# AI4REALNET/network-distributed-q-learning

Hardware: NVIDIA B200
Metric: switch_agent_decisions_per_sec (higher is better)
Workload: dtype f64

## Files before the change

network-distributed-q-learning_b200/csrc/sfl_core.cuh:

```cuda
#pragma once
#include <stdint.h>
#include "switchfl_b200.h"

#if defined(__CUDACC__) && !defined(SFL_HOST_EMUL)
#define SFL_DEV 1
#define SFL_FN __device__ __forceinline__
#define SFL_NI __device__ __forceinline__
#define SFL_RARE __device__ __noinline__
#define SFL_NU _Pragma("unroll 1")
#define SFL_U4 _Pragma("unroll 4")
#define SFL_UA _Pragma("unroll")
#else
#define SFL_DEV 0
#include <math.h>
#include <string.h>
#define SFL_FN inline
#define SFL_NI inline
#define SFL_RARE inline
#define SFL_NU
#define SFL_U4
#define SFL_UA
struct int4 { int x, y, z, w; };
struct int2 { int x, y; };
static inline int4 make_int4(int x, int y, int z, int w) { int4 r = {x, y, z, w}; return r; }
// ... 101 lines not shown
  RO<int> dist;
  RO<int8_t> qinit;
};

struct Layout {
  int T, S, NP, NT, a_max, q_cap, q_stride, pend_cap;
  unsigned off_tra, off_trb, off_pend, off_sem, off_rewards, off_sws, off_q;
  unsigned off_rng;
  unsigned long long env_stride;
};

struct EnvHdr {
  int elapsed, episode, step_counter, num_malf;
  int terminated, truncated, need_reset, halted;
  int err, q_rows, pending_fin, cur_dec;
  int act_cursor, ev_cursor, n_dec_logged, n_tick_logged;
  int n_ep_logged, q_init_on, aborted, cur_train;
  unsigned long long active_mask, malf_prev_mask, at_dest_mask, done_mask;
  unsigned long long decisions, ticks, train_ticks;
  double cum_reward;
  int last_next_sw;
  int eps_tag;
  unsigned eps_z, eps_w;
  unsigned long long forced_stops, stop_actions, arrived_trains;
  int dec_t, dec_go;
  unsigned long long ph[6], ph_t0;
};

struct SwS { int ninter, pad; double eps_pow; };
enum { HM_ACTIVE = 0, HM_MALF = 1, HM_DEST = 2, HM_DONE = 3 };

struct RunArgs {
  int mode, max_ticks, n_envs, trace_sem;
  int dec_cap, tick_cap, ep_cap, act_cap, ev_cap, max_steps, q_init_on, phase_clock;
  unsigned hot_bytes, env_smem, tail_hot, pad2;
  char *state;
  const sfl_hparams *hp;
  sfl_env_counters *counters;
  sfl_dec_rec *trace_dec; sfl_tick_rec *trace_tick; int4 *trace_sem_buf;
  sfl_ep_rec *ep_log; int *ep_delay;
  sfl_step_rec *step_out;
  double *sq_q; long long *sq_d; int *sq_c;
  const int8_t *replay_act; const int *replay_ev;
  const double *eval_q;
};

struct KArgs { DevMap m; Layout L; RunArgs ra; };
#define SFL_K const KArgs &K
#define c_m (K.m)
#define c_L (K.L)
#define c_ra (K.ra)

#if SFL_DEV
extern __shared__ __align__(16) char g_smem[];
typedef unsigned hot_t;
SFL_FN char *hot_ptr(hot_t o) { return g_smem + o; }
#else
typedef char *hot_t;
SFL_FN char *hot_ptr(hot_t o) { return o; }
#endif

template <bool TH, bool SQ_ = false> struct EnvT {
  static const bool SQ = SQ_;
  static const bool EVQ = false;
  static const bool HOT_TAIL = TH;
  static const int NW = 1;
  const KArgs *kp;
  hot_t hot;
  char *gb;
  SFL_FN EnvHdr *h() const { return (EnvHdr *)hot_ptr(hot); }
  SFL_FN int4 *tra() const { return (int4 *)(hot_ptr(hot) + kp->L.off_tra); }
  SFL_FN int4 *trb() const { return (int4 *)(hot_ptr(hot) + kp->L.off_trb); }
  SFL_FN char *tail() const { return TH ? hot_ptr(hot) : gb; }
  SFL_FN int2 *pend() const { return (int2 *)(tail() + kp->L.off_pend); }
  SFL_FN int4 *sem() const { return (int4 *)(tail() + kp->L.off_sem); }
  SFL_FN int *rewards() const { return (int *)(tail() + kp->L.off_rewards); }
  SFL_FN SwS *sws() const { return (SwS *)(tail() + kp->L.off_sws); }
  SFL_FN double *q() const { return (double *)(gb + kp->L.off_q); }
  hot_t own;
  SFL_FN uint8_t *own_ptr() const { return (uint8_t *)hot_ptr(own); }
  SFL_FN int owner(int p) const { return TH ? sem()[p].z : (int)(int8_t)own_ptr()[p]; }
  SFL_FN void sem_put(int p, int4 r) const { sem()[p] = r; if (!TH) own_ptr()[p] = (uint8_t)r.z; }
  SFL_FN void sem_drop(int p) const { sem()[p].z = -1; if (!TH) own_ptr()[p] = 0xFFu; }
  SFL_FN unsigned long long &hw0(int m) const {
    EnvHdr *x = h();
    return m == HM_ACTIVE ? x->active_mask : m == HM_MALF ? x->malf_prev_mask : m == HM_DEST ? x->at_dest_mask : x->done_mask;
  }
  SFL_FN unsigned long long *hw1(int m) const { return (unsigned long long *)(hot_ptr(hot) + sizeof(EnvHdr)) + m; }
};
template <bool TH, bool SQ_ = false> struct EnvW : EnvT<TH, SQ_> { static const int NW = 2; };
template <class Base> struct EnvEval : Base { static const bool EVQ = true; };
template <bool TH, bool SQ, int NW, bool EVQ = false> struct EnvOf { typedef EnvT<TH, SQ> type; };
template <bool TH, bool SQ> struct EnvOf<TH, SQ, 2, false> { typedef EnvW<TH, SQ> type; };
template <bool TH, int NW> struct EnvOf<TH, false, NW, true> { typedef EnvEval<typename EnvOf<TH, false, NW>::type> type; };

template <class Env> SFL_FN TSet<Env::NW> tset(const Env &e, int m) {
  TSet<Env::NW> s; s.w[0] = e.hw0(m); if (Env::NW > 1) s.w[Env::NW - 1] = *e.hw1(m); return s;
}
template <class Env> SFL_FN void tset_put(const Env &e, int m, const TSet<Env::NW> &s) { e.hw0(m) = s.w[0]; if (Env::NW > 1) *e.hw1(m) = s.w[Env::NW - 1]; }
template <class Env> SFL_FN int tset_any(const Env &e, int m) { return Env::NW == 1 ? e.hw0(m) != 0ull : (e.hw0(m) | *e.hw1(m)) != 0ull; }
template <class Env> SFL_FN int tset_pop(const Env &e, int m) { TSet<Env::NW> s = tset(e, m); const int t = s.pop(); tset_put(e, m, s); return t; }
template <class Env> SFL_FN void tset_add(const Env &e, int m, int t) {
  if (Env::NW > 1 && t >= 64) *e.hw1(m) |= 1ull << (t & 63); else e.hw0(m) |= 1ull << t;
}



struct Scratch {
  const KArgs *kp;
  hot_t base;
  SFL_FN int4 *tmp() const { return (int4 *)hot_ptr(base); }
  SFL_FN int4 *rng() const { return (int4 *)(hot_ptr(base) + 16 * kp->L.T); }
  SFL_FN int *inj() const { return (int *)(hot_ptr(base) + 16 * kp->L.T); }
  SFL_FN int8_t *occ() const { return (int8_t *)(hot_ptr(base) + 32 * kp->L.T); }
  SFL_FN uint8_t *blk() const { return (uint8_t *)(hot_ptr(base) + 33 * kp->L.T); }
};
#if SFL_DEV
__host__
#endif
SFL_FN unsigned scratch_bytes(int T) { return (unsigned)(32 * T + ((2 * T + 15) / 16) * 16); }

struct Hp {
  hot_t o;
  SFL_FN const sfl_hparams *operator->() const { return (const sfl_hparams *)hot_ptr(o); }
};

#if SFL_DEV
SFL_FN unsigned long long sm_clock() { return (unsigned long long)clock64(); }
#else
SFL_FN unsigned long long sm_clock() { return 0ull; }
#endif
enum { PH_TICK = 0, PH_OBSERVE = 1, PH_ACT = 2, PH_APPLY = 3, PH_UPDATE = 4, PH_RESET = 5 };
#define SFL_PHASE_START(h) do { if (TRACE && c_ra.phase_clock) (h)->ph_t0 = sm_clock(); } while (0)
#define SFL_PHASE_MARK(h, i) do { if (TRACE && c_ra.phase_clock) { const unsigned long long t_ = sm_clock(); (h)->ph[i] += t_ - (h)->ph_t0; (h)->ph_t0 = t_; } } while (0)

enum { K_LEARN = 0, K_GREEDY = 1, K_FULL = 2 };
template <int KIND> SFL_FN int run_mode(SFL_K) { return KIND == K_LEARN ? (int)SFL_MODE_LEARN : KIND == K_GREEDY ? (int)SFL_MODE_GREEDY : c_ra.mode; }

struct U4 { unsigned x, y, z, w; };
SFL_FN unsigned mulhi32(unsigned a, unsigned b) { return (unsigned)(((unsigned long long)a * b) >> 32); }
SFL_FN U4 philox4x32(unsigned c0, unsigned c1, unsigned c2, unsigned c3, unsigned k0, unsigned k1) {
  SFL_NU
  for (int i = 0; i < 10; i++) {
    unsigned h0 = mulhi32(0xD2511F53u, c0), l0 = 0xD2511F53u * c0;
    unsigned h1 = mulhi32(0xCD9E8D57u, c2), l1 = 0xCD9E8D57u * c2;
    unsigned n0 = h1 ^ c1 ^ k0, n2 = h0 ^ c3 ^ k1;
    c0 = n0; c1 = l1; c2 = n2; c3 = l0;
    k0 += 0x9E3779B9u; k1 += 0xBB67AE85u;
  }
  U4 r = {c0, c1, c2, c3};
  return r;
}

struct Pcg {
  unsigned long long s_hi, s_lo, i_hi, i_lo;
  unsigned has32, u32, pad0, pad1;
};
#define SFL_PCG_BYTES 48

SFL_FN void pcg_step(Pcg &g) {
  const unsigned long long M_HI = 0x2360ED051FC65DA4ull, M_LO = 0x4385DF649FCCF645ull;
  const unsigned long long lo = g.s_lo * M_LO;
  const unsigned long long hi = mulhi64(g.s_lo, M_LO) + g.s_lo * M_HI + g.s_hi * M_LO;
  g.s_lo = lo + g.i_lo;
  g.s_hi = hi + g.i_hi + (g.s_lo < lo ? 1ull : 0ull);
}
// ... 88 lines not shown
#define SFL_MT_N 624
#define SFL_MT_M 397
SFL_FN unsigned mt_temper(unsigned y) {
  y ^= y >> 11;
  y ^= (y << 7) & 0x9D2C5680u;
  y ^= (y << 15) & 0xEFC60000u;
  return y ^ (y >> 18);
}
template <int G> SFL_FN int mt_seed(unsigned *key, unsigned long long seed, const Grp<G> &g) {
  if (seed >> 32) return 0;
  if (g.gl == 0) {
    unsigned s = (unsigned)seed;
    SFL_NU
    for (int i = 0; i < SFL_MT_N; i++) { key[i] = s; s = 1812433253u * (s ^ (s >> 30)) + (unsigned)(i + 1); }
  }
  g.sync();
  return 1;
}
template <int G> SFL_FN void mt_twist(unsigned *key, unsigned *out, const Grp<G> &g) {
  SFL_NU
  for (int base = 0; base < SFL_MT_N; base += G) {
    const int i = base + g.gl;
    unsigned v = 0u;
    if (i < SFL_MT_N) {
      const unsigned y = (key[i] & 0x80000000u) | (key[i + 1 == SFL_MT_N ? 0 : i + 1] & 0x7FFFFFFFu);
      v = key[i < SFL_MT_N - SFL_MT_M ? i + SFL_MT_M : i - (SFL_MT_N - SFL_MT_M)] ^ (y >> 1) ^ ((0u - (y & 1u)) & 0x9908B0DFu);
    }
    g.sync();
    if (i < SFL_MT_N) key[i] = v;
    g.sync();
  }
  for (int i = g.gl; i < SFL_MT_N; i += G) out[i] = mt_temper(key[i]);
  g.sync();
}
template <int G> SFL_FN unsigned mt_next(unsigned *key, unsigned *out, int &pos, const Grp<G> &g) {
  if (pos == SFL_MT_N) { mt_twist(key, out, g); pos = 0; }
  return out[pos++];
}
template <int G> SFL_FN unsigned mt_masked(unsigned *key, unsigned *out, int &pos, const Grp<G> &g, unsigned rng) {
  if (!rng) return 0u;
  unsigned mask = rng;
  mask |= mask >> 1; mask |= mask >> 2; mask |= mask >> 4; mask |= mask >> 8; mask |= mask >> 16;
  unsigned v;
  SFL_NU
  do v = mt_next(key, out, pos, g) & mask; while (v > rng);
  return v;
}
template <int G> SFL_FN int malf_schedule_env(unsigned long long seed, unsigned long long hit_below, int lo, int hi, int T, int steps,
                                              int *ev, int ev_cap, unsigned *key, unsigned *out, const Grp<G> &g) {
  if (!mt_seed(key, seed, g)) return -1;
  int n = 0, pos = SFL_MT_N;
  const unsigned rng = (unsigned)hi - (unsigned)lo;
  SFL_NU
  for (int tick = 1; hit_below && tick <= steps; tick++) {
    SFL_NU
    for (int t = 0; t < T; t++) {
      const unsigned a = mt_next(key, out, pos, g), b = mt_next(key, out, pos, g);
      if ((((unsigned long long)(a >> 5) << 26) | (b >> 6)) >= hit_below) continue;
      const int dur = lo + (int)mt_masked(key, out, pos, g, rng) + 1;
      if (g.gl == 0 && n < ev_cap) { ev[3 * n] = tick; ev[3 * n + 1] = t; ev[3 * n + 2] = dur; }
      n++;
    }
  }
  if (g.gl == 0 && n < ev_cap) ev[3 * n] = -1;
  return n;
}

struct Mv { int cell, dir, valid; };
SFL_FN unsigned mv_entry(SFL_K, int cell, int dir) { return c_m.move[(size_t)cell * 4 + dir]; }
SFL_FN int mv_valid(unsigned e, int action) { return (e >> (3 * action)) & 1; }
SFL_FN Mv mv_apply(SFL_K, unsigned e, int action, int cell) {
  unsigned f = (e >> (3 * action)) & 7u;
  int nd = (int)(f >> 1);
  int delta = (nd & 1) ? (2 - nd) : (nd - 1) * c_m.Wp;
  Mv r;
  r.cell = (e & 0x8000u) ? cell + delta : cell;
  r.dir = nd; r.valid = (int)(f & 1u);
  return r;
}
SFL_FN Mv check_action(SFL_K, int action, int cell, int dir) { return mv_apply(K, mv_entry(K, cell, dir), action, cell); }

SFL_FN int is_moving(int a) { return a >= A_LEFT && a <= A_RIGHT; }

template <class Env>
SFL_FN int tr_state(Env e, int t) { return (e.tra()[t].y >> 8) & 0xFF; }
template <class Env>
SFL_FN int rule_port(Env e, int port, int me, int now, int blocking_type) {
  int4 r;
  if (Env::HOT_TAIL) {
    r = e.sem()[port];
    if (r.z < 0 || r.z == me || r.x > now || r.x + r.y < now) return 0;
  } else {
    const int holder = e.owner(port);
    if (holder < 0 || holder == me) return 0;
    r = e.sem()[port];
    if (r.x > now || r.x + r.y < now) return 0;
  }
  if (r.w == blocking_type) return 1;
  return tr_state(e, r.z) == ST_MALF;
}
template <class Env>
SFL_FN int port_blocked(Env e, int next_port, int out_port, int me, int now) {
  if (next_port >= 0) {
    if (rule_port(e, next_port, me, now, SEM_OUT)) return 1;
    return rule_port(e, out_port, me, now, SEM_IN);
  }
  return rule_port(e, out_port, me, now, SEM_OUT);
}

template <class Env>
SFL_RARE void q_insert(SFL_K, Env e, const Hp hp, unsigned key, double *row) {
  *(unsigned long long *)row = (unsigned long long)key + 1ull;
  e.h()->q_rows++;
  unsigned per_port = (unsigned)(c_L.NT * 48);
  int port = (int)(key / per_port);
  int A = c_m.sw[c_m.port[port].w].y;
  double dq = hp->default_q;
  SFL_NU
  for (int a = 0; a < A; a++) row[1 + a] = dq;
  if (c_ra.q_init_on) {
    unsigned rem = key - (unsigned)port * per_port;
    int tgt = (int)(rem / 48u), semb = (int)((rem % 48u) / 3u);
    int qi = c_m.qinit[port * c_L.NT + tgt];
    if (qi >= 0 && semb != 0) row[1 + (qi & 15)] = (qi & 16) ? 1000.0 : 500.0;
  }
}

template <class Env>
SFL_NI double *q_row(SFL_K, Env e, const Hp hp, unsigned key) {
  if (Env::SQ) return c_ra.sq_q + (size_t)key * c_L.a_max;
  unsigned mask = (unsigned)c_L.q_cap - 1u;
  unsigned i = (key * 2654435761u) >> 7;
  SFL_NU
  for (int probe = 0; probe < c_L.q_cap; probe++) {
    i &= mask;
    double *row = e.q() + (size_t)i * c_L.q_stride;
    unsigned long long k = *(unsigned long long *)row;
    if (k == (unsigned long long)key + 1ull) return row + 1;
    if (k == 0ull) {
      if (e.h()->q_rows >= c_L.q_cap - 1) break;
      q_insert(K, e, hp, key, row);
      return row + 1;
    }
    i++;
  }
  e.h()->err |= SFL_ERR_Q_FULL;
  return e.q() + 1;
}

#if SFL_DEV
SFL_FN void shared_add(long long *d, int *c, long long v) { atomicAdd((unsigned long long *)d, (unsigned long long)v); atomicAdd(c, 1); }
#else
SFL_FN void shared_add(long long *d, int *c, long long v) { *d += v; *c += 1; }
#endif

SFL_FN double lr_pow(double rate, int n) {
  double r = 1.0, b = rate;
  SFL_NU
  for (; n > 0; n >>= 1) { if (n & 1) r = dmul(r, b); b = dmul(b, b); }
  return r;
}

SFL_FN double td_value(double q, double lr, double reward, double gamma, double mq, int bootstrap) {
  const double one_m = dadd(1.0, -lr);
  return bootstrap ? dadd(dmul(one_m, q), dmul(lr, dadd(reward, dmul(gamma, mq)))) : dadd(dmul(one_m, q), dmul(lr, reward));
}

template <class Env>
SFL_NI void q_update(SFL_K, Env e, const Hp hp, unsigned key, int action, double reward,
                     const double *next_row, int prev_sw, int next_sw) {
  double *row = q_row(K, e, hp, key);
  double lr = hp->lr;
  if (hp->lr_decay_rate != 1.0) lr = dmul(lr, lr_pow(hp->lr_decay_rate, e.sws()[prev_sw].ninter));
  const double q = row[action];
  double mq = 0.0;
  if (next_sw != prev_sw && next_row) {
    int A = c_m.sw[next_sw].y;
    mq = next_row[0];
    SFL_NU
    for (int a = 1; a < A; a++) { const double v = next_row[a]; mq = v > mq ? v : mq; }
// ... 73 lines not shown
      if (r.z < 0 || r.x > now) e.sem()[unique] = make_int4(now, d_ot, h, SEM_OUT);
      if (far_port != source && far_port != out_port && far_port != unique) {
        r = e.sem()[far_port];
        if (r.z < 0 || r.w == SEM_IN || r.x > now) e.sem()[far_port] = make_int4(now, d_ot + up.y + 1, h, SEM_IN);
      }
    }
    if (target != source && target != out_port) {
      r = e.sem()[target];
      if (r.z < 0 || r.w == SEM_OUT || r.x > now) e.sem()[target] = make_int4(now, d_ot + 1, h, SEM_OUT);
    }
  } else {
    int4 r;
    if (e.owner(out_port) < 0) e.sem_put(out_port, make_int4(now, 3, h, SEM_OUT));
    else { r = e.sem()[out_port]; if (r.w == SEM_OUT || r.x > now) e.sem_put(out_port, make_int4(now, 3, h, r.w)); }
    int d_ot = c_m.port[out_port].y;
    if (e.owner(target) < 0) e.sem_put(target, make_int4(now, d_ot + 1, h, SEM_IN));
    else { r = e.sem()[target]; if (r.w == SEM_IN || r.x > now) e.sem_put(target, make_int4(now, d_ot + 1, h, r.w)); }
    int unique = c_m.port[target].z;
    if (unique >= 0) {
      int4 up = c_m.port[unique];
      int far_port = up.x;
      if (unique != source && unique != out_port && unique != target) {
        r = e.sem()[unique];
        if (e.owner(unique) < 0 || r.w == SEM_OUT || r.x > now) e.sem_put(unique, make_int4(now, d_ot + 1, h, SEM_OUT));
      }
      r = e.sem()[unique];
      if (e.owner(unique) < 0 || r.x > now) e.sem_put(unique, make_int4(now, d_ot, h, SEM_OUT));
      if (far_port != source && far_port != out_port && far_port != unique) {
        r = e.sem()[far_port];
        if (e.owner(far_port) < 0 || r.w == SEM_IN || r.x > now) e.sem_put(far_port, make_int4(now, d_ot + up.y + 1, h, SEM_IN));
      }
    }
    if (target != source && target != out_port) {
      r = e.sem()[target];
      if (e.owner(target) < 0 || r.w == SEM_OUT || r.x > now) e.sem_put(target, make_int4(now, d_ot + 1, h, SEM_OUT));
    }
  }
}

template <class Env>
SFL_FN int delay_at(SFL_K, Env e, int tgt_index, int cell, int dir, int now, int la) {
  int d = c_m.dist[((size_t)tgt_index * (c_m.Hp * c_m.Wp) + cell) * 4 + dir];
  if (d >= SFL_INF_DIST) { e.h()->err |= SFL_ERR_INF_DISTANCE; d = 0; }
  return now - la + d;
}

template <int KIND, class Env>
SFL_FN void finish_decision(SFL_K, Env e, const Hp hp, int env_id) {
  const bool TRACE = KIND == K_FULL;
  const int mode = run_mode<KIND>(K);
  EnvHdr *h = e.h();
  SFL_PHASE_START(h);
  if (mode == SFL_MODE_LEARN || mode == SFL_MODE_REPLAY) {
    TSet<Env::NW> fresh = tset(e, HM_DONE).andnot(tset(e, HM_DEST));
    SFL_NU
    while (fresh.any()) {
      int t = fresh.pop();
      tset_add(e, HM_DEST, t);
      int4 b = e.trb()[t];
      int n = (b.y >> 16) & 0xFF;
      SFL_NU
      for (int i = 0; i < n; i++) {
        int2 pe = e.pend()[t * c_L.pend_cap + i];
        q_update(K, e, hp, (unsigned)pe.x, (pe.y >> 24) & 15, 1000.0, nullptr, (pe.y >> 12) & 0xFFF, -1);
      }
      b.y &= 0xFFFF;
      e.trb()[t] = b;
    }
    SwS *ss = e.sws() + h->pending_fin;
    ss->ninter++;
    ss->eps_pow = dmul(ss->eps_pow, hp->epsilon_decay_rate);
  }
  h->pending_fin = -1;
  SFL_PHASE_MARK(h, PH_UPDATE);
  if (h->step_counter > c_ra.max_steps) h->truncated = 1;
  if (TRACE) {
    if (c_ra.trace_dec && h->cur_dec >= 0 && h->cur_dec < c_ra.dec_cap) {
      sfl_dec_rec *rec = c_ra.trace_dec + (size_t)env_id * c_ra.dec_cap + h->cur_dec;
      rec->arrived = h->done_mask; rec->arrived_hi = Env::NW > 1 ? *e.hw1(HM_DONE) : 0ull;
      rec->done = h->terminated | (h->truncated << 1);
      if (c_ra.trace_sem_buf) {
        int4 *dst = c_ra.trace_sem_buf + ((size_t)env_id * c_ra.dec_cap + h->cur_dec) * c_L.NP;
        SFL_NU
        for (int p = 0; p < c_L.NP; p++) { int4 r = e.sem()[p]; r.y += r.x; dst[p] = r; }
      }
    }
    h->cur_dec = -1;
  }
}

template <int G, class Env>
SFL_FN int observe_bits(SFL_K, Env e, const Grp<G> &g, const int on, const int t) {
  const int now = e.h()->elapsed;
  const int s = on ? (e.trb()[t].y & 0xFFFF) : 0;
  const int4 sw = c_m.sw[s];
  unsigned bits = 0;
  SFL_UA
  for (int base = 0; base < 8; base += G) {
    const int j = base + g.gl;
    int b = 0;
    if (on && j < 8 && (j & 3) < sw.x) {
      const int port = sw.z + (j & 3);
      b = (j & 4) ? rule_port(e, port, t, now, SEM_IN) : rule_port(e, c_m.port[port].x, t, now, SEM_OUT);
    }
    bits |= (g.ballot(b) & 0xFFu) << base;
  }
  return (int)(~(bits | (bits >> 4)) & ((1u << sw.x) - 1u));
}

struct Obs { int s, P, A, p0, a0, cur, semb, mask, ok; unsigned key; };
template <class Env>
SFL_FN Obs observe(SFL_K, Env e, int t, int now, const int4 ta, const int4 tb, const int semb_pre = -1) {
  Obs ob;
  ob.s = tb.y & 0xFFFF;
  const int4 sw = c_m.sw[ob.s];
  ob.P = sw.x; ob.A = sw.y; ob.p0 = sw.z; ob.a0 = sw.w;
  const int4 tr0 = c_m.train0[t], tr1 = c_m.train1[t];
  const int my_port = (int)((unsigned)ta.w >> 16);
  const int dist_now = c_m.dist[((size_t)tr0.w * (c_m.Hp * c_m.Wp) + ta.x) * 4 + (ta.y & 0xFF)];
  int semb = semb_pre;
  if (semb_pre < 0) {
    semb = 0;
    SFL_NU
    for (int k = 0; k < ob.P; k++)
      if (!port_blocked(e, c_m.port[ob.p0 + k].x, ob.p0 + k, t, now)) semb |= 1 << k;
  }
  ob.semb = semb;
  ob.cur = my_port - ob.p0;
  ob.ok = ob.cur >= 0 && ob.cur < ob.P;
  ob.key = 0u; ob.mask = 0;
  if (!ob.ok) return ob;
  int delay = now - tr1.y + dist_now;
  if (dist_now >= SFL_INF_DIST) { e.h()->err |= SFL_ERR_INF_DISTANCE; delay = now - tr1.y; }
  int level = delay <= 0 ? 0 : (delay <= (tr1.y - tr1.x) * 20 ? 1 : 2);
  ob.key = (((unsigned)(ob.p0 + ob.cur) * c_L.NT + tr0.w) * 16u + semb) * 3u + level;
  const int4 px = c_m.pexit[ob.p0 + ob.cur];
  int mask = 1 << (ob.A - 1);
  {
    int ex[3] = {px.y, px.z, px.w};
#if SFL_DEV
#pragma unroll
#endif
    for (int i = 0; i < 3; i++) if (i < px.x && ((semb >> ((ex[i] >> 4) & 3)) & 1)) mask |= 1 << (ex[i] & 15);
  }
  ob.mask = mask;
  return ob;
}

template <int KIND, class Env>
SFL_FN void decide(SFL_K, Env e, const Hp hp, int env_id, int t, const int semb_pre = -1) {
  const bool TRACE = KIND == K_FULL;
  const int mode = run_mode<KIND>(K);
  EnvHdr *h = e.h();
  const int now = h->elapsed;
  SFL_PHASE_START(h);
  int4 ta = e.tra()[t], tb = e.trb()[t];
  const int learning = mode == SFL_MODE_LEARN || mode == SFL_MODE_REPLAY;
  const int s_early = tb.y & 0xFFFF;
  const int reward_in = e.rewards()[s_early * c_L.T + t];
  double eps_pow = 1.0;
  int ninter = 0;
  if (mode == SFL_MODE_LEARN) {
    eps_pow = e.sws()[s_early].eps_pow;
    if (KIND == K_FULL && c_L.off_rng) ninter = e.sws()[s_early].ninter;
  }
  int2 pend0 = make_int2(0, -1);
  if (learning && ((tb.y >> 16) & 0xFF)) pend0 = e.pend()[t * c_L.pend_cap];
// ... 77 lines not shown
    if (pl >= SFL_PLAN_CAP) { h->err |= SFL_ERR_PLAN_FULL; pl = SFL_PLAN_CAP - 1; }
    plan = ((plan << 4) | A_STOP) & 0xFFFFu; pl++;
  } else { plan = A_FWD | ((unsigned)move2 << 4); pl = 2; }
  ta.z = (int)plan | (pl << 16);
  e.tra()[t] = ta;
  int all_blocked = 1;
  if ((plan & 0xFu) == A_STOP) {
    if (moving) all_blocked = port_blocked(e, next_port, out_port, t, now);
    else all_blocked = (mask == (1 << (A - 1)));
  }
  int cell = pos, d2 = dir;
  {
    unsigned pp = plan;
    SFL_NU
    for (int i = 0; i < pl; i++, pp >>= 4) {
      int a = pp & 0xF;
      if (a != A_STOP) { Mv c = check_action(K, a, cell, d2); cell = c.cell; d2 = c.dir; }
    }
  }
  int curr = delay_at(K, e, tr0.w, cell, d2, now, tr1.y);
  int reward_out = tb.z - curr;
  if (!all_blocked && (plan & 0xFu) == A_STOP) reward_out -= 1300;
  e.rewards()[next_switch * c_L.T + t] = reward_out;
  tb.z = curr;
  h->step_counter++;
  SFL_PHASE_MARK(h, PH_APPLY);
  if (learning) {
    int n = (tb.y >> 16) & 0xFF;
    int2 *pend = e.pend() + t * c_L.pend_cap;
    int hit = -1, same = -1;
    SFL_NU
    for (int i = 0; i < n; i++) {
      int nsw = (i ? pend[i].y : pend0.y) & 0xFFF;
      if (nsw == s && hit < 0) hit = i;
    }
    if (hit >= 0) {
      int2 pe = hit ? pend[hit] : pend0;
      const int prev_sw = (pe.y >> 12) & 0xFFF;
      if (prev_sw != s && !my_row) my_row = q_row(K, e, hp, key);
      q_update(K, e, hp, (unsigned)pe.x, (pe.y >> 24) & 15, (double)reward_in, my_row, prev_sw, s);
      SFL_NU
      for (int j = hit; j + 1 < n; j++) pend[j] = pend[j + 1];
      n--;
    }
    int meta = next_switch | (s << 12) | (action << 24);
    SFL_NU
    for (int i = 0; i < n; i++) if ((pend[i].y & 0xFFF) == next_switch) same = i;
    if (same >= 0) pend[same] = make_int2((int)key, meta);
    else if (n >= c_L.pend_cap) h->err |= SFL_ERR_PEND_FULL;
    else { pend[n] = make_int2((int)key, meta); n++; }
    tb.y = (tb.y & 0xFFFF) | (n << 16);
  }
  e.trb()[t] = tb;
  SFL_PHASE_MARK(h, PH_UPDATE);
  h->cum_reward += (double)reward_in;
  if (TRACE) {
    if (c_ra.trace_dec) {
      h->cur_dec = h->n_dec_logged;
      if (h->n_dec_logged < c_ra.dec_cap) {
        sfl_dec_rec *rec = c_ra.trace_dec + (size_t)env_id * c_ra.dec_cap + h->n_dec_logged;
        rec->ep = h->episode; rec->tick = now; rec->sw = s; rec->train = t; rec->key = key; rec->mask = mask;
        rec->action = action; rec->next_sw = next_switch; rec->reward = reward_in; rec->done = 0; rec->arrived = 0;
        rec->arrived_hi = 0;
      }
      h->n_dec_logged++;
    }
  }
  if (TRACE) h->last_next_sw = next_switch;
  h->decisions++;
  if (mask == (1 << (A - 1))) h->forced_stops++;
  if (action == A - 1) h->stop_actions++;
  h->pending_fin = s;
}

template <int G, class Env>
SFL_RARE void env_reset(SFL_K, Env e, const Grp<G> &g, int on) {
  EnvHdr *h = e.h();
  const int T = on ? c_L.T : 0, NP = on ? c_L.NP : 0;
  SFL_NU
  for (int t = g.gl; t < T; t += G) {
    int4 tr0 = c_m.train0[t], tr1 = c_m.train1[t];
    e.tra()[t] = make_int4(-1, tr0.y | (ST_WAITING << 8) | (0 << 16) | (A_NONE << 24), 0, (int)((unsigned)tr1.z << 16));
    int4 b = e.trb()[t];
    e.trb()[t] = make_int4(b.x, 0xFFFF, c_m.init_delay[t], 0);
  }
  SFL_NU
  for (int p = g.gl; p < NP; p += G) e.sem_put(p, make_int4(0, 0, -1, 0));
  SFL_NU
  for (int i = g.gl; i < c_L.S * T; i += G) e.rewards()[i] = 0;
  g.sync();
  if (on && g.gl == 0) {
    SFL_NU
    for (int t = 0; t < T; t++) {
      int4 tr1 = c_m.train1[t];
      e.sem_put(tr1.z, make_int4(tr1.x - 2, tr1.w + 2, t, SEM_IN));
    }
    h->elapsed = 0; h->step_counter = 0; h->num_malf = 0; h->terminated = 0; h->truncated = 0; h->need_reset = 0;
    h->pending_fin = -1; h->cur_dec = -1; h->ev_cursor = 0; h->active_mask = 0; h->malf_prev_mask = 0; h->at_dest_mask = 0;
    h->eps_tag = -1;
    h->done_mask = 0; h->cum_reward = 0.0;
    if (Env::NW > 1) { SFL_UA for (int m = 0; m < 4; m++) *e.hw1(m) = 0ull; }
  }
  g.sync();
}

template <int NW> struct TickRegs {
  int elapsed, ended, rng_blk;
  TSet<NW> active, done;
  unsigned ticks, train_ticks;
};

SFL_FN int malf_stage2(const Hp hp, int now, int t) {
  const U4 u = philox4x32((unsigned)now, (unsigned)t, 0xA11Eu, 0u, (unsigned)hp->seed, (unsigned)(hp->seed >> 32));
  if (u.x >= hp->malf_thr2) return 0;
  return hp->malf_min + (int)(((unsigned long long)u.y * (unsigned)(hp->malf_max - hp->malf_min + 1)) >> 32) + 1;
}

template <int G, int KIND, bool ONE, class Env>
SFL_FN void env_tick(SFL_K, Env e, Scratch sc, const Hp hp, int env_id, const Grp<G> &g, TickRegs<Env::NW> &R, const int live) {
  const bool TRACE = KIND == K_FULL;
  EnvHdr *h = e.h();
  const int Tw = c_L.T;
  const int T = live ? Tw : 0;
  const int now = R.elapsed + 1;
  const int replay_ev = KIND != K_LEARN && c_ra.replay_ev != 0;
  const unsigned thr = live ? hp->malf_threshold : 0u;
  if (replay_ev) {
    SFL_NU
    for (int t = g.gl; t < T; t += G) sc.inj()[t] = 0;
    g.sync();
    if (live && g.gl == 0) {
      const int *ev = c_ra.replay_ev + (size_t)env_id * c_ra.ev_cap * 3;
      int c = h->ev_cursor;
      SFL_NU
      while (c < c_ra.ev_cap && ev[c * 3] >= 0 && ev[c * 3] <= now) { if (ev[c * 3] == now) sc.inj()[ev[c * 3 + 1]] = ev[c * 3 + 2]; c++; }
      h->ev_cursor = c;
    }
    g.sync();
  }
  const int fresh_rng = !replay_ev && thr && (now >> 4) != R.rng_blk;
  const unsigned coarse = (thr >> 24) + ((thr & 0xFFFFFFu) ? 1u : 0u);
  SFL_NU
  for (int t = g.gl, once_ = 1; t < T && (!ONE || once_); t += G, once_ = 0) {
    int4 ta = e.tra()[t];
    const int p = ta.x, d = ta.y & 0xFF, st = (ta.y >> 8) & 0xFF;
    int saved = (ta.y >> 16) & 0xFF, prev_act = (ta.y >> 24) & 0xFF;
    unsigned plan = (unsigned)ta.z & 0xFFFFu;
    int pl = ta.z >> 16, mc = ta.w & 0xFFFF;
    int dur = 0;
    if (replay_ev) dur = sc.inj()[t];
    else if (thr) {
      if (fresh_rng) {
        U4 u = philox4x32((unsigned)(now >> 4), (unsigned)t, 0xA11Fu, 0u, (unsigned)hp->seed, (unsigned)(hp->seed >> 32));
        sc.rng()[t] = make_int4((int)u.x, (int)u.y, (int)u.z, (int)u.w);
      }
      if (((const uint8_t *)&sc.rng()[t])[now & 15] < coarse) dur = malf_stage2(hp, now, t);
    }
    if (mc == 0 && dur > 0) mc = dur;
    int src, dst, ecell = -1, nd = d, act = A_NOTHING, a = A_NOTHING, flags = 0;
    if (st == ST_DONE) { src = dst = -1 - t; }
    else {
      int pp = p, dd = d;
      if (p < 0) { const int4 tr0 = c_m.train0[t]; pp = tr0.x; dd = tr0.y; }
      const unsigned me = mv_entry(K, pp, dd);
      if (pl == 0) a = A_FWD;
      else { a = plan & 0xF; prev_act = a; plan >>= 4; pl--; }
      if (p >= 0) { Mv c = mv_apply(K, me, a, p); ecell = c.valid ? c.cell : p; flags = 1 | (c.valid ? 2 : 0); }
      act = a;
      if (st == ST_WAITING) act = A_NOTHING;
      if ((act == A_LEFT || act == A_RIGHT) && !mv_valid(me, act)) act = A_FWD;
      if (is_moving(act) && !mv_valid(me, act)) act = A_STOP;
      if (is_moving(act) && !saved) saved = act;
      const int upd = (mc == 0) && act != A_STOP;
      int ncell = p;
      if (p < 0) { if (saved) { ncell = pp; nd = dd; } }
      else if (saved && upd) { Mv c = mv_apply(K, me, saved, p); if (c.valid) { ncell = c.cell; nd = c.dir; } act = saved; }
      src = p >= 0 ? p : -1 - t;
      dst = ncell >= 0 ? ncell : src;
    }
    ta.y = d | (st << 8) | (saved << 16) | (prev_act << 24);
    ta.z = (int)plan | (pl << 16);
    ta.w = (ta.w & (int)0xFFFF0000) | mc;
    e.tra()[t] = ta;
    sc.tmp()[t] = make_int4(src, dst, ecell, nd | (act << 8) | (a << 16) | (flags << 24));
  }
  if (fresh_rng) R.rng_blk = now >> 4;
  g.sync();
  TSet<Env::NW> chain;
  chain.clear();
  SFL_NU
  for (int base = 0; base < (ONE ? 1 : Tw); base += (ONE ? 1 : G)) {
    const int t = base + g.gl;
    int follows = 0;
    if (t < T) {
      int4 m = sc.tmp()[t];
      int s = m.x, d = m.y;
      int wants = d != s, blocked = !wants, occ = -1;
      if (wants) {
        SFL_NU
        for (int k = 0; k < T; k++) {
          const int2 o = *(const int2 *)&sc.tmp()[k];
          occ = o.x == d ? k : occ;
          blocked |= (o.y == d) & (o.y != o.x) & (k < t);
        }
        if (occ >= 0) { int2 o = *(const int2 *)&sc.tmp()[occ]; if (o.y == s && o.y != o.x) blocked = 1; }
      }
      sc.occ()[t] = (int8_t)occ; sc.blk()[t] = (uint8_t)blocked;
      follows = !blocked && occ >= 0;
    }
    chain.or_ballot(g.ballot(follows), base);
  }
  g.sync();
  if (g.wany(chain.any())) {
    SFL_NU
    for (int iter = 0; iter < Tw; iter++) {
      int changed = 0;
      if (chain.any()) {
        SFL_NU
        for (int t = g.gl, once_ = 1; t < T && (!ONE || once_); t += G, once_ = 0) {
          int occ = sc.occ()[t];
          if (!sc.blk()[t] && occ >= 0 && ((volatile uint8_t *)sc.blk())[occ]) { sc.blk()[t] = 1; changed = 1; }
        }
      }
      g.sync();
      if (!g.wany(changed)) break;
    }
  }
  TSet<Env::NW> done_bits, malf_bits, stopped_bits, depart_bits, active;
  done_bits.clear(); malf_bits.clear(); stopped_bits.clear(); depart_bits.clear(); active.clear();
  SFL_NU
  for (int base = 0; base < (ONE ? 1 : Tw); base += (ONE ? 1 : G)) {
    const int t = base + g.gl;
    int f_done = 0, f_malf = 0, f_stop = 0, f_dep = 0, f_act = 0;
    if (t < T) {
      int4 ta = e.tra()[t];
      const int4 m = sc.tmp()[t];
      int p = ta.x, d = ta.y & 0xFF;
      const int st = (ta.y >> 8) & 0xFF;
      int saved = (ta.y >> 16) & 0xFF;
      const int prev_act = (ta.y >> 24) & 0xFF;
      unsigned plan = (unsigned)ta.z & 0xFFFFu;
      int pl = ta.z >> 16, mc = ta.w & 0xFFFF, next_port = (int)((unsigned)ta.w >> 16);
      const int act = (m.w >> 8) & 0xFF, popped = (m.w >> 16) & 0xFF, fl = (m.w >> 24) & 0xFF;
      const int wants = m.y != m.x;
      const int in_malf = mc > 0, allowed = !in_malf && wants && !sc.blk()[t];
      const int4 tr0 = c_m.train0[t];
      const int ed = c_m.train1[t].x;
      const int ed_reached = now >= ed, stop_given = act == A_STOP, valid_move = is_moving(act) && allowed, conflict = !allowed;
      int nxt = st;
      switch (st) {
        case ST_WAITING: if (in_malf) nxt = ST_MALF_OFF; else if (ed_reached) nxt = ST_READY; break;
        case ST_READY: if (in_malf) nxt = ST_MALF_OFF; else if (valid_move) nxt = ST_MOVING; break;
        case ST_MALF_OFF:
          if (!in_malf) { if (ed_reached) nxt = valid_move ? ST_MOVING : ST_STOPPED; else nxt = ST_WAITING; }
          break;
        case ST_MOVING: if (in_malf) nxt = ST_MALF; else if (stop_given || conflict) nxt = ST_STOPPED; break;
        case ST_STOPPED: if (in_malf) nxt = ST_MALF; else if (valid_move) nxt = ST_MOVING; break;
        case ST_MALF: if (!in_malf && valid_move) nxt = ST_MOVING; else if (!in_malf && (stop_given || conflict)) nxt = ST_STOPPED; break;
        default: break;
      }
      if (nxt >= ST_MOVING && nxt <= ST_MALF) {
        if (st <= ST_MALF_OFF) { p = tr0.x; d = tr0.y; }
        else if (allowed) { p = m.y; d = m.w & 0xFF; if (p == tr0.z) nxt = ST_DONE; }
      }
      if (nxt == ST_DONE) p = -1;
      if (mc > 0) mc--;
      if (p >= 0) saved = 0;
      f_done = nxt == ST_DONE; f_malf = mc != 0; f_stop = nxt == ST_STOPPED || nxt == ST_MALF; f_dep = now == ed - 2;
      if (TRACE) {
        if (c_ra.trace_tick && h->n_tick_logged < c_ra.tick_cap) {
          sfl_tick_rec *rec = c_ra.trace_tick + ((size_t)env_id * c_ra.tick_cap + h->n_tick_logged) * T + t;
          rec->pos = p; rec->dir = (int8_t)d; rec->state = (int8_t)nxt; rec->malf = (int16_t)mc;
        }
      }
      if ((fl & 1) && (fl & 2) && m.z != p && popped != A_STOP) {
        if (pl >= SFL_PLAN_CAP) { h->err |= SFL_ERR_PLAN_FULL; pl = SFL_PLAN_CAP - 1; }
        plan = ((plan << 4) | (unsigned)popped) & 0xFFFFu; pl++;
        if (c_m.cell_switch[m.z] >= 0) {
          int src_port = (int)((unsigned)e.trb()[t].x >> 16);
          if (src_port != 0xFFFF) next_port = src_port;
        }
      }
      if (p >= 0 && nxt != ST_WAITING) {
        int peek = pl ? (int)(plan & 0xF) : A_FWD;
        Mv c = check_action(K, peek, p, d);
        int s = c_m.cell_switch[c.cell];
        if (s >= 0) {
          int ok = 1;
          if (nxt == ST_MOVING || nxt == ST_READY) { }
          else if ((nxt == ST_STOPPED || nxt == ST_MALF) && prev_act == A_STOP) { }
          else if (nxt == ST_STOPPED || nxt == ST_MALF) s = c_m.port[next_port].w;
          else ok = 0;
          if (ok) { ((uint16_t *)&e.trb()[t].y)[0] = (uint16_t)s; f_act = 1; }
        }
      }
      ta.x = p;
      ta.y = d | (nxt << 8) | (saved << 16) | (prev_act << 24);
      ta.z = (int)plan | (pl << 16);
      ta.w = mc | (next_port << 16);
      e.tra()[t] = ta;
    }
    done_bits.or_ballot(g.ballot(f_done), base);
    malf_bits.or_ballot(g.ballot(f_malf), base);
    stopped_bits.or_ballot(g.ballot(f_stop), base);
    depart_bits.or_ballot(g.ballot(f_dep), base);
    active.or_ballot(g.ballot(f_act), base);
  }
  const int ended = live && (done_bits.all(Tw) || now >= c_m.max_episode_steps);
  const TSet<Env::NW> prev_done = R.done;
  const int release = done_bits.andnot(prev_done).any() || ended;
  if (g.wany(release)) {
    const int NP = release ? c_L.NP : 0;
    SFL_NU
    for (int p = g.gl; p < NP; p += G) {
      int tr = e.owner(p);
      if (tr >= 0 && (ended || done_bits.test(tr))) e.sem_drop(p);
    }
  }
  if (g.wany(depart_bits.any())) {
    g.sync();
    if (depart_bits.any() && g.gl == 0) {
      TSet<Env::NW> b = depart_bits;
      SFL_NU
      while (b.any()) {
        int t = b.pop();
        int4 tr1 = c_m.train1[t];
        e.sem_put((int)((unsigned)e.tra()[t].w >> 16), make_int4(tr1.x - 2, tr1.w + 2, t, SEM_IN));
      }
    }
  }
  if (g.wany(stopped_bits.any())) {
    g.sync();
    const int NP = stopped_bits.any() ? c_L.NP : 0;
    SFL_NU
    for (int p = g.gl; p < NP; p += G) {
      if (Env::HOT_TAIL) {
        int4 r = e.sem()[p];
        if (r.z >= 0 && stopped_bits.test(r.z)) e.sem()[p].x = now;
      } else {
        const int holder = e.owner(p);
        if (holder >= 0 && stopped_bits.test(holder)) e.sem()[p].x = now;
      }
    }
    g.sync();
    if (stopped_bits.any() && g.gl == 0) {
      TSet<Env::NW> b = stopped_bits;
      SFL_NU
      while (b.any()) {
        int t = b.pop();
        int4 ta = e.tra()[t];
        if (((ta.y >> 8) & 0xFF) == ST_MALF) {
          int port = (int)((unsigned)ta.w >> 16);
          if (e.owner(port) < 0) e.sem_put(port, make_int4(now, c_m.train1[t].w, t, SEM_IN));
        }
      }
    }
  }
  if (live && g.gl == 0) {
    h->elapsed = now;
    const TSet<Env::NW> malf_prev = tset(e, HM_MALF);
    const TSet<Env::NW> new_malf = malf_bits.andnot(malf_prev);
    if (new_malf.any()) h->num_malf += new_malf.popc();
    if (!(malf_bits == malf_prev)) tset_put(e, HM_MALF, malf_bits);
    if (!(done_bits == prev_done)) tset_put(e, HM_DONE, done_bits);
    if (ended) h->terminated = 1;
    if (active.any()) tset_put(e, HM_ACTIVE, active);
    if (TRACE) { if (c_ra.trace_tick) h->n_tick_logged++; }
  }
  R.elapsed = now; R.ended = ended; R.active = active; R.done = done_bits;
  if (live) { R.ticks++; R.train_ticks += (unsigned)(T - prev_done.popc()); }
  g.sync();
}

template <class Env>
SFL_RARE void episode_end(SFL_K, Env e, int env_id) {
  EnvHdr *h = e.h();
  if (c_ra.ep_log && h->n_ep_logged < c_ra.ep_cap) {
    const TSet<Env::NW> done = tset(e, HM_DONE);
    sfl_ep_rec *rec = c_ra.ep_log + (size_t)env_id * c_ra.ep_cap + h->n_ep_logged;
    rec->cum_reward = h->cum_reward; rec->decisions = h->step_counter; rec->arrived = done.popc();
    rec->num_malfunctions = h->num_malf; rec->ticks = h->elapsed; rec->arrived_mask = done.w[0];
    rec->arrived_mask_hi = Env::NW > 1 ? done.w[Env::NW - 1] : 0ull;
    if (c_ra.ep_delay) {
      int *d = c_ra.ep_delay + ((size_t)env_id * c_ra.ep_cap + h->n_ep_logged) * c_L.T;
      SFL_NU
      for (int t = 0; t < c_L.T; t++) d[t] = e.trb()[t].z;
    }
  }
  h->arrived_trains += (unsigned)tset(e, HM_DONE).popc();
  h->n_ep_logged++;
  h->episode++;
  h->need_reset = 1;
}

template <class Env>
SFL_FN void step_report(SFL_K, Env e, int env_id, int t) {
  EnvHdr *h = e.h();
  sfl_step_rec *o = c_ra.step_out + env_id;
  o->pending = 0; o->sw = -1; o->train = -1; o->key = 0u; o->mask = 0;
  if (t >= 0) {
    const int4 ta = e.tra()[t], tb = e.trb()[t];
    const Obs ob = observe(K, e, t, h->elapsed, ta, tb);
    if (!ob.ok) { h->err |= SFL_ERR_NO_TRAIN_AT_SWITCH; h->aborted++; h->truncated = 1; }
    else {
      o->pending = 1; o->sw = ob.s; o->train = t; o->key = ob.key; o->mask = ob.mask;
      SFL_NU
      for (int k = 0; k < c_L.T; k++) o->rewards[k] = e.rewards()[ob.s * c_L.T + k];
      h->cur_train = t;
    }
  }
  o->done = h->terminated | (h->truncated << 1);
  o->elapsed = h->elapsed; o->last_next_sw = h->last_next_sw; o->arrived = h->done_mask;
  o->arrived_hi = Env::NW > 1 ? *e.hw1(HM_DONE) : 0ull;
}

template <int G, int KIND, bool TH, bool SQ, bool ONE, int NW = 1, bool EVQ = false>
SFL_FN void env_run(SFL_K, int env_id, unsigned stage, char *host_scratch) {
  const bool TRACE = KIND == K_FULL;
  const Grp<G> g;
  const int valid = env_id < c_ra.n_envs;
  if (!valid) env_id = 0;
  char *gbase = c_ra.state + (size_t)env_id * c_L.env_stride;
  const unsigned hot_bytes = valid ? c_ra.hot_bytes : 0u;
  typename EnvOf<TH, SQ, NW, EVQ>::type e;
  Hp hp;
  Scratch sc;
  e.kp = &K; sc.kp = &K;
  e.gb = gbase;
#if SFL_DEV
  {
    char *smem = g_smem + stage;
    SFL_NU
    for (unsigned o = g.gl * 16u; o < hot_bytes; o += G * 16u) *(int4 *)(smem + o) = *(const int4 *)(gbase + o);
    if (valid) {
      SFL_NU
      for (unsigned o = g.gl * 16u; o < (unsigned)sizeof(sfl_hparams); o += G * 16u)
        *(int4 *)(smem + c_ra.hot_bytes + o) = *(const int4 *)((const char *)(c_ra.hp + env_id) + o);
// ... 117 lines not shown
```

Measured before the change: 396.6 million.

## Replace per-tick semaphore refresh scan with per-train stop timestamps

Instead of walking every port each tick to refresh the start time of semaphores held by stopped or malfunctioning trains, each train records its last stop tick in trb().w. Readers compute an effective start time as max(start, stop_tick) when checking blocking. This removes an O(NP) loop and two group syncs from the tick path whenever any train is stopped. In exchange, every rule_port check does an extra indirect load of the holder's stop tick, and stopped trains write trb each tick.

```diff
diff --git a/network-distributed-q-learning_b200/csrc/sfl_core.cuh b/network-distributed-q-learning_b200/csrc/sfl_core.cuh
--- a/network-distributed-q-learning_b200/csrc/sfl_core.cuh
+++ b/network-distributed-q-learning_b200/csrc/sfl_core.cuh
@@ -207,6 +207,7 @@
   SFL_FN int owner(int p) const { return TH ? sem()[p].z : (int)(int8_t)own_ptr()[p]; }
   SFL_FN void sem_put(int p, int4 r) const { sem()[p] = r; if (!TH) own_ptr()[p] = (uint8_t)r.z; }
   SFL_FN void sem_drop(int p) const { sem()[p].z = -1; if (!TH) own_ptr()[p] = 0xFFu; }
+  SFL_FN int stop_tick(int t) const { return trb()[t].w; }
   SFL_FN unsigned long long &hw0(int m) const {
     EnvHdr *x = h();
     return m == HM_ACTIVE ? x->active_mask : m == HM_MALF ? x->malf_prev_mask : m == HM_DEST ? x->at_dest_mask : x->done_mask;
@@ -461,20 +462,25 @@
 
 SFL_FN int is_moving(int a) { return a >= A_LEFT && a <= A_RIGHT; }
 
+#define SFL_NO_STOP (-0x7FFFFFFF - 1)
+SFL_FN int t0_eff(int t0, int stop_tick) { return t0 > stop_tick ? t0 : stop_tick; }
 template <class Env>
 SFL_FN int tr_state(Env e, int t) { return (e.tra()[t].y >> 8) & 0xFF; }
 template <class Env>
 SFL_FN int rule_port(Env e, int port, int me, int now, int blocking_type) {
   int4 r;
+  int stamp;
   if (Env::HOT_TAIL) {
     r = e.sem()[port];
-    if (r.z < 0 || r.z == me || r.x > now || r.x + r.y < now) return 0;
+    if (r.z < 0 || r.z == me) return 0;
+    stamp = e.stop_tick(r.z);
   } else {
     const int holder = e.owner(port);
     if (holder < 0 || holder == me) return 0;
     r = e.sem()[port];
-    if (r.x > now || r.x + r.y < now) return 0;
-  }
+    stamp = e.stop_tick(holder);
+  }
+  if (r.x > now || t0_eff(r.x, stamp) + r.y < now) return 0;
   if (r.w == blocking_type) return 1;
   return tr_state(e, r.z) == ST_MALF;
 }
@@ -714,7 +720,11 @@
       if (c_ra.trace_sem_buf) {
         int4 *dst = c_ra.trace_sem_buf + ((size_t)env_id * c_ra.dec_cap + h->cur_dec) * c_L.NP;
         SFL_NU
-        for (int p = 0; p < c_L.NP; p++) { int4 r = e.sem()[p]; r.y += r.x; dst[p] = r; }
+        for (int p = 0; p < c_L.NP; p++) {
+          int4 r = e.sem()[p];
+          if (r.z >= 0) r.x = t0_eff(r.x, e.stop_tick(r.z));
+          r.y += r.x; dst[p] = r;
+        }
       }
     }
     h->cur_dec = -1;
@@ -958,7 +968,7 @@
     int4 tr0 = c_m.train0[t], tr1 = c_m.train1[t];
     e.tra()[t] = make_int4(-1, tr0.y | (ST_WAITING << 8) | (0 << 16) | (A_NONE << 24), 0, (int)((unsigned)tr1.z << 16));
     int4 b = e.trb()[t];
-    e.trb()[t] = make_int4(b.x, 0xFFFF, c_m.init_delay[t], 0);
+    e.trb()[t] = make_int4(b.x, 0xFFFF, c_m.init_delay[t], SFL_NO_STOP);
   }
   SFL_NU
   for (int p = g.gl; p < NP; p += G) e.sem_put(p, make_int4(0, 0, -1, 0));
@@ -1102,12 +1112,12 @@
       if (!g.wany(changed)) break;
     }
   }
-  TSet<Env::NW> done_bits, malf_bits, stopped_bits, depart_bits, active;
-  done_bits.clear(); malf_bits.clear(); stopped_bits.clear(); depart_bits.clear(); active.clear();
+  TSet<Env::NW> done_bits, malf_bits, broken_bits, depart_bits, active;
+  done_bits.clear(); malf_bits.clear(); broken_bits.clear(); depart_bits.clear(); active.clear();
   SFL_NU
   for (int base = 0; base < (ONE ? 1 : Tw); base += (ONE ? 1 : G)) {
     const int t = base + g.gl;
-    int f_done = 0, f_malf = 0, f_stop = 0, f_dep = 0, f_act = 0;
+    int f_done = 0, f_malf = 0, f_broken = 0, f_dep = 0, f_act = 0;
     if (t < T) {
       int4 ta = e.tra()[t];
       const int4 m = sc.tmp()[t];
@@ -1142,7 +1152,8 @@
       if (nxt == ST_DONE) p = -1;
       if (mc > 0) mc--;
       if (p >= 0) saved = 0;
-      f_done = nxt == ST_DONE; f_malf = mc != 0; f_stop = nxt == ST_STOPPED || nxt == ST_MALF; f_dep = now == ed - 2;
+      f_done = nxt == ST_DONE; f_malf = mc != 0; f_broken = nxt == ST_MALF; f_dep = now == ed - 2;
+      if (nxt == ST_STOPPED || nxt == ST_MALF) e.trb()[t].w = now;
       if (TRACE) {
         if (c_ra.trace_tick && h->n_tick_logged < c_ra.tick_cap) {
           sfl_tick_rec *rec = c_ra.trace_tick + ((size_t)env_id * c_ra.tick_cap + h->n_tick_logged) * T + t;
@@ -1178,7 +1189,7 @@
     }
     done_bits.or_ballot(g.ballot(f_done), base);
     malf_bits.or_ballot(g.ballot(f_malf), base);
-    stopped_bits.or_ballot(g.ballot(f_stop), base);
+    broken_bits.or_ballot(g.ballot(f_broken), base);
     depart_bits.or_ballot(g.ballot(f_dep), base);
     active.or_ballot(g.ballot(f_act), base);
   }
@@ -1193,9 +1204,9 @@
       if (tr >= 0 && (ended || done_bits.test(tr))) e.sem_drop(p);
     }
   }
-  if (g.wany(depart_bits.any())) {
+  if (g.wany(depart_bits.any() || broken_bits.any())) {
     g.sync();
-    if (depart_bits.any() && g.gl == 0) {
+    if (g.gl == 0) {
       TSet<Env::NW> b = depart_bits;
       SFL_NU
       while (b.any()) {
@@ -1203,32 +1214,12 @@
         int4 tr1 = c_m.train1[t];
         e.sem_put((int)((unsigned)e.tra()[t].w >> 16), make_int4(tr1.x - 2, tr1.w + 2, t, SEM_IN));
       }
-    }
-  }
-  if (g.wany(stopped_bits.any())) {
-    g.sync();
-    const int NP = stopped_bits.any() ? c_L.NP : 0;
-    SFL_NU
-    for (int p = g.gl; p < NP; p += G) {
-      if (Env::HOT_TAIL) {
-        int4 r = e.sem()[p];
-        if (r.z >= 0 && stopped_bits.test(r.z)) e.sem()[p].x = now;
-      } else {
-        const int holder = e.owner(p);
-        if (holder >= 0 && stopped_bits.test(holder)) e.sem()[p].x = now;
-      }
-    }
-    g.sync();
-    if (stopped_bits.any() && g.gl == 0) {
-      TSet<Env::NW> b = stopped_bits;
+      b = broken_bits;
       SFL_NU
       while (b.any()) {
         int t = b.pop();
-        int4 ta = e.tra()[t];
-        if (((ta.y >> 8) & 0xFF) == ST_MALF) {
-          int port = (int)((unsigned)ta.w >> 16);
-          if (e.owner(port) < 0) e.sem_put(port, make_int4(now, c_m.train1[t].w, t, SEM_IN));
-        }
+        int port = (int)((unsigned)e.tra()[t].w >> 16);
+        if (e.owner(port) < 0) e.sem_put(port, make_int4(now, c_m.train1[t].w, t, SEM_IN));
       }
     }
   }
```

Result: faster. 424.3 million (median of 6 runs) (+7.0%).
